# adelacvg/diff-vits

Measured on AMD Instinct MI355X. Metric: mel_frames_per_sec_50step_dpmsolver, higher is better.
Workload: dtype bf16x3 (bf16 MFMA operands split hi+lo, 3 products, fp32 accumulate / fp32 activations); 1 GPU; B=8/GPU, C=80, T=1024, L=256, 50-step DPM-Solver++(2M) multistep, UNet1DConditionModel (128, 256, 384, 512), seeded random-init weights; global_batch=8, concurrent_sub_batches_per_gpu=1, rccl_world_size=1, parallelism=dp1 (batch-sharded, RCCL broadcast of conditioning + all-gather of mels)

## Files before the change

diff-vits_amd/csrc/dv_common.h:

```cpp
#pragma once
#include <hip/hip_runtime.h>
#include <stdint.h>

typedef unsigned short bf16_t;

enum { DV_ZERO_PAGE_BYTES = 32768 };
enum { EPI_STORE = 0, EPI_RESIDUAL = 1, EPI_GEGLU = 2, EPI_STORE_NCT = 3 };
enum { UP_NONE = 0, UP_X2 = 1, UP_SIZE = 2 };

struct GemmSeg {
  const bf16_t* a0_hi; const bf16_t* a0_lo;
  const bf16_t* a1_hi; const bf16_t* a1_lo;
  int c0, c1;
  int taps;
  int pad;
  int nkt;
};

struct GnxParams {
  unsigned long long* xchg;
  unsigned* status;
  const float* gamma; const float* beta;
  const float* tscale; const float* tshift; int ld_t;
  int groups; float eps; int silu;
// ... 97 lines not shown
struct ChainFFParams {
  int M, C, T;
  int Tv;
  const bf16_t* a_hi; const bf16_t* a_lo;
  const float* rowstat; float ln_eps;
  const bf16_t* wg_hi; const bf16_t* wg_lo; const float* bg; const float* ug;
  const bf16_t* wm_hi; const bf16_t* wm_lo; const float* bm;
  const float* res;
  float* out; float* stats16;
  bf16_t* out_hi; bf16_t* out_lo;
  GnxParams gnx;
};
bool chain_ff_supported(const ChainFFParams& p, int precision);
int chain_ff_gnx_plan(const ChainFFParams& p, int n_cu);
hipError_t launch_chain_ff(const ChainFFParams& p, int precision, hipStream_t st);

struct FFSplitParams {
  int M, C, T;
  int rows;
  int Tv;
  int nspl;
  const bf16_t* a_hi; const bf16_t* a_lo;
  const float* rowstat; float ln_eps;
  const bf16_t* wg_hi; const bf16_t* wg_lo; const float* bg; const float* ug;
  const bf16_t* wm_hi; const bf16_t* wm_lo; const float* bm;
  const float* res;
  float* out; float* stats16;
  bf16_t* out_hi; bf16_t* out_lo;
  float* xbuf;
  unsigned long long* flags;
// ... 154 lines not shown
```

diff-vits_amd/csrc/engine.hip:

```cpp
#include "../../include/dvits_hip.h"
#include "dv_common.h"

#include <atomic>
#include <cmath>
#include <cstdarg>
#include <cstdio>
#include <cstdlib>
#include <cstring>
#include <functional>
#include <map>
#include <memory>
#include <string>
#include <type_traits>
#include <vector>

static thread_local char g_err[1024] = "";
int dv_fail(int code, const char* fmt, ...) {
  va_list ap;
  va_start(ap, fmt);
  vsnprintf(g_err, sizeof(g_err), fmt, ap);
  va_end(ap);
  return code;
}
extern "C" const char* dv_last_error(void) { return g_err; }
// ... 584 lines not shown
    Planes y, sy, sr;
    if (!gnx_offer(prod, nn, &y, &sy, &sr)) return;
    const bool cat = nn.skip.C > 0;
    out.n_hi = y.hi; out.n_lo = y.lo; out.n_pre = nn.pre;
    if (cat) { out.sn_hi = sy.hi; out.sn_lo = sy.lo; out.sr_hi = sr.hi; out.sr_lo = sr.lo; }
    const bool fp32_unread = cat && nn.raw && !u->keep_intermediates;
    if (nn.raw && !prod.out_hi) out_planes(prod, out);
    if (fp32_unread && cat_drop_fp32) prod.out = nullptr;
  }
  template <class P> void out_planes(P& prod, Act& out) {
    Planes pl = alloc_planes((size_t)prod.M * out.C);
    out.pl_hi = pl.hi; out.pl_lo = pl.lo; prod.out_hi = pl.hi; prod.out_lo = pl.lo;
  }
  bool ff_split_on = [] { const char* e = getenv("DVITS_FF_SPLIT"); return !(e && e[0] == '0'); }();
  bool chain_ff_on = [] { const char* e = getenv("DVITS_CHAIN_FF"); return !(e && e[0] == '0'); }();
  bool chain_split_on = [] { const char* e = getenv("DVITS_CHAIN_SPLIT"); return !(e && e[0] == '0'); }();
  bool chain_xsplit_on = [] { const char* e = getenv("DVITS_CHAIN_XSPLIT"); return !(e && e[0] == '0'); }();
  bool qkv_split_on = [] { const char* e = getenv("DVITS_QKV_SPLIT"); return !(e && e[0] == '0'); }();
  int qkv_split_min_wg = [] { const char* e = getenv("DVITS_QKV_SPLIT_MIN_WG"); return e ? atoi(e) : 96; }();
  int qkv_split_min_c = [] { const char* e = getenv("DVITS_QKV_SPLIT_MIN_C"); return e ? atoi(e) : 256; }();
  bool qkv_xa_on = [] { const char* e = getenv("DVITS_QKV_XA"); return !(e && e[0] == '0'); }();
  int qkv_xa_min_c = [] { const char* e = getenv("DVITS_QKV_XA_MIN_C"); return e ? atoi(e) : 256; }();
  int ff_split_min_wg = [] { const char* e = getenv("DVITS_FF_SPLIT_MIN_WG"); return e ? atoi(e) : 96; }();
  bool gnx_ff_on = [] { const char* e = getenv("DVITS_GNX_FF"); return !(e && e[0] == '0'); }();
  bool cat_drop_fp32 = [] { const char* e = getenv("DVITS_GNX_CONCAT_KEEP_FP32"); return !(e && e[0] == '1'); }();

  int conv3_min_tiles = [] { const char* e = getenv("DVITS_CONV3_MIN_TILES"); return e ? atoi(e) : 64; }();
  int conv3_route(const GemmParams& g) const {
    if (arena.exact || autotune_on() || prec != DV_PREC_BF16X3) return 0;
    GemmParams t = g;
// ... 338 lines not shown
    b.w_q2 = pack(tb + "q2", C, C, {{tb + "attn2.to_q.weight", 0, C, 1, C, 0, 0, tb + "norm2.weight", 0}},
                  {{"", "", tb + "attn2.to_q.weight", tb + "norm2.bias", C, C, 0, 0}});
    b.w_o2 = pack(tb + "out2", C, C, {{tb + "attn2.to_out.0.weight", 0, C, 1, C, 0, 0, "", 0}},
                  {{tb + "attn2.to_out.0.bias", "", "", "", C, 0, 0, 0}});
    b.w_gg = pack(tb + "geglu", 8 * C, C, {{tb + "ff.net.0.proj.weight", 0, C, 1, C, 0, 0, tb + "norm3.weight", 1}},
                  {{tb + "ff.net.0.proj.bias", "", tb + "ff.net.0.proj.weight", tb + "norm3.bias", 8 * C, C, 0, 1}});
    b.merged_ffproj = merge_ff && fuse_ln && !u->keep_intermediates;
    b.w_ff = b.merged_ffproj ? b.w_gg : pack(tb + "ffout", C, 4 * C, {{tb + "ff.net.2.weight", 0, 4 * C, 1, 4 * C, 0, 0, "", 0}},
                                             {{tb + "ff.net.2.bias", "", "", "", C, 0, 0, 0}});
    b.w_out = b.merged_ffproj ? b.w_gg : pack(p + "proj_out", C, C, {{p + "proj_out.weight", 1, C, 1, C, 0, 0, "", 0}},
                                              {{p + "proj_out.bias", "", "", "", C, 0, 0, 0}});
    if (!b.w_in || !b.w_qkv || !b.w_o1 || !b.w_q2 || !b.w_o2 || !b.w_gg || !b.w_ff || !b.w_out) return Act{};

    float* h3 = nullptr;
    LnIn l3;
    if (chain_ok(b.Tp, C) && x.stat16) {
      if (!(frag(b.w_in) && frag(b.w_qkv) && frag(b.w_o1) && frag(b.w_q2))) return Act{};
      float* h = nullptr;
      const Planes ao = xf_head(ops, b, h);
      if (!xf_tail(ops, b, h, ao, h3, l3)) return Act{};
    } else h3 = xf_attention_gemms(ops, b, l3);
    return xf_ff(ops, b, h3, l3, want_planes);
  }

  Planes xf_head(std::vector<OpFn>& ops, const Xf& b, float*& h) {
    const int C = b.C, Tn = b.Tn, Tp = b.Tp, M = b.M;
    h = alloc((size_t)M * C);
    const int dh = C / u->cfg.num_heads;
    const bool sa_frag = attn_frag_on && !arena.exact && C % u->cfg.num_heads == 0 && dh % 16 == 0 && dh <= 64;
    float* qkv = alloc((size_t)M * (sa_frag ? 1 : 3) * C);
    Planes kf, vf;
    if (sa_frag) { kf = alloc_planes((size_t)M * C); vf = alloc_planes((size_t)M * C); }
    ChainParams cp{};
    cp.M = M; cp.C = C; cp.T = Tp; cp.Tv = Tn; cp.amode = 1;
    cp.x = b.x.p; cp.stat16 = b.x.stat16; cp.gamma = W(b.p + "norm.weight"); cp.beta = W(b.p + "norm.bias"); cp.gn_eps = 1e-6f;
    cp.groups = u->cfg.norm_num_groups;
    cp.w1_hi = b.w_in->fhi; cp.w1_lo = b.w_in->flo; cp.Kp1 = b.w_in->Kp; cp.b1 = b.w_in->bias; cp.res = nullptr; cp.out1 = h;
// ... 14 lines not shown
    if (sa_frag) {
      AttnFragParams a{};
      a.q = qkv; a.ldq = C;
      a.kf_hi = kf.hi; a.kf_lo = kf.lo; a.vf_hi = vf.hi; a.vf_lo = vf.lo;
      const int nT = Tp / 32;
      a.k_b = nT * (C / 16); a.k_h = dh / 16; a.k_t = C / 16;
      a.v_b = nT * (C / 32) * 2; a.v_h = 0; a.v_t = (C / 32) * 2; a.v_kb = 1; a.v_nb = 2; a.self_layout = 1;
      a.bias = nullptr; a.bias_ld = 0;
      ao = attention_frag(ops, a, Tp, Tn, C);
      release(kf); release(vf);
    } else ao = attention(ops, qkv, 3 * C, qkv + C, qkv + 2 * C, 3 * C, nullptr, Tp, Tn, C, Tp);
    release(qkv);
    return ao;
  }

  bool xf_tail(std::vector<OpFn>& ops, const Xf& b, float* h, Planes ao, float*& h3, LnIn& l3) {
    const int C = b.C, M = b.M;
    if (xa_ok(b.Tp, C) && cross_frag.count(b.p)) {
      if (!frag(b.w_o2)) return false;
      float* h2 = alloc((size_t)M * C);
      h3 = alloc((size_t)M * C);
      l3 = ln_planes(M, C);
      xf_xattn_chain(ops, b, h, ao, h2, h3, l3);
      release(ao); release(h);
      probe(b.tb + "attn1", h2, b.Tn, C);
      release(h2);
      probe(b.tb + "attn2", h3, b.Tn, C);
      return true;
    }
    float* h2 = alloc((size_t)M * C);
    float* q2 = alloc((size_t)M * C);
    ChainParams cp = tail_chain(b, h, ao, h2);
    cp.out2 = q2;
    {
      const int rbs = M / 32, cus = n_cu > 0 ? n_cu : 256, nsg = C / 128;
      cp.nsplit = (chain_split_on && nsg >= 2 && rbs * nsg <= cus) ? nsg : 1;
    }
    const int n_qflags = qkv_split_flags(cp);
// ... 3 lines not shown
    if (!split) chain(ops, cp, "to_out+res+LN+to_q");
    release(ao); release(h);
    probe(b.tb + "attn1", h2, b.Tn, C);
    h3 = cross_attention_out(ops, b, q2, h2, l3);
    return true;
  }
  ChainParams tail_chain(const Xf& b, float* h, Planes ao, float* h2) {
    ChainParams cp{};
    cp.M = b.M; cp.C = b.C; cp.T = b.Tp; cp.Tv = b.Tn; cp.amode = 0;
    cp.a_hi = ao.hi; cp.a_lo = ao.lo;
    cp.w1_hi = b.w_o1->fhi; cp.w1_lo = b.w_o1->flo; cp.Kp1 = b.w_o1->Kp; cp.b1 = b.w_o1->bias; cp.res = h; cp.out1 = h2;
    cp.w2_hi = b.w_q2->fhi; cp.w2_lo = b.w_q2->flo; cp.Kp2 = b.w_q2->Kp; cp.b2 = b.w_q2->bias; cp.u2 = b.w_q2->u;
    cp.passes = 1; cp.out2 = nullptr; cp.ldo2 = b.C; cp.ln_eps = 1e-5f;
    return cp;
  }
  void xf_xattn_chain(std::vector<OpFn>& ops, const Xf& b, float* h, Planes ao, float* h2, float* h3, const LnIn& l3) {
    const int C = b.C, Tp = b.Tp, M = b.M;
    const XFrag& xf = cross_frag[b.p];
    ChainParams cp = tail_chain(b, h, ao, h2);
    cp.xa_kf_hi = xf.kf_hi; cp.xa_kf_lo = xf.kf_lo; cp.xa_vf_hi = xf.vf_hi; cp.xa_vf_lo = xf.vf_lo; cp.xa_bias = xbias;
    cp.xa_nT = (L + 31) / 32; cp.xa_d = C / u->cfg.num_heads;
    cp.xa_qscale = (1.0f / sqrtf((float)cp.xa_d)) * 1.44269504088896340736f;
    cp.w3_hi = b.w_o2->fhi; cp.w3_lo = b.w_o2->flo; cp.b3 = b.w_o2->bias;
    cp.out3 = h3; cp.out3_hi = l3.pl.hi; cp.out3_lo = l3.pl.lo; cp.rowstat3 = l3.stat;
    {
      const int rbs = M / 32, cus = n_cu > 0 ? n_cu : 256;
      if (chain_xsplit_on && C == 256 && rbs * 2 <= cus && rbs <= 4096 && (dry || u->sk_tickets)) {
        cp.nsplit = 2;
        cp.xs_buf = alloc((size_t)rbs * 2 * C * 32);
        cp.xs_ticket = dry ? reinterpret_cast<unsigned*>(0x1000) : u->sk_tickets;
      }
    }
    ChainParams cq = cp;
    cq.nsplit = 1; cq.xs_buf = nullptr; cq.xs_ticket = nullptr;
    const double xattn_flops = 4.0 * B * u->cfg.num_heads * (double)Tp * L * cp.xa_d + 2.0 * (double)M * C * C;
    const int n_wg = (M / 64) * (C / 64);
    bool split_xa = qkv_split_on && qkv_xa_on && C >= qkv_xa_min_c && handover_ok() && !autotune_on() &&
                    Tp % 64 == 0 && (M / 64) % 8 == 0 && n_wg <= n_cu && n_wg >= qkv_split_min_wg && u->cfg.num_heads == 8 &&
                    gnx_used + (size_t)2 * n_wg <= dv_unet::GNX_POOL;
    Planes oxa;
    if (split_xa) {
      oxa = alloc_planes((size_t)M * C);
      cq.qs_o_hi = oxa.hi; cq.qs_o_lo = oxa.lo;
      split_xa = qkv_split(ops, cq, strf("to_out+res+LN+to_q+xattn+to_out+res (%d wg / 64 rows) M=%d C=%d", C / 64, M, C), xattn_flops);
      if (!split_xa) release(oxa);
    }
    if (!split_xa)
      chain(ops, cp, cp.nsplit == 2 ? "to_out+res+LN+to_q+xattn(2 wg)+to_out+res" : "to_out+res+LN+to_q+xattn+to_out+res", xattn_flops);
    if (cp.xs_buf) release(cp.xs_buf);
    if (split_xa) release(oxa);
  }

  float* xf_attention_gemms(std::vector<OpFn>& ops, const Xf& b, LnIn& l3) {
    const int C = b.C, Tn = b.Tn, Tp = b.Tp, M = b.M;
    float* h = alloc((size_t)M * C);
    LnIn l1;
    {
      GemmParams g = gp_base(Tn, M, C);
      g.out = h; l1 = ln_produce(g, M, C);
      Planes gn;
      if (b.x.n_hi && b.x.n_pre == b.p + "norm") { gn.hi = b.x.n_hi; gn.lo = b.x.n_lo; }
// ... 36 lines not shown
    Planes ao;
    if (attn_frag_on && !arena.exact && cross_frag.count(b.p)) ao = cross_attention_frag(ops, b.p, q2, Tp, C);
    else ao = attention(ops, q2, C, kv, kv + C, 2 * C, mask_bias, Tp, L, C);
    release(q2);
    float* h3 = alloc((size_t)M * C);
    {
      GemmParams g = gp_base(b.Tn, M, C); g.seg[0] = seg(ao, C, Planes{}, 0, 1, 0);
      g.epi = EPI_RESIDUAL; g.res = h2; g.out = h3; l3 = ln_produce(g, M, C);
      gemm(ops, g, b.w_o2, C);
    }
    release(ao); release(h2);
    probe(b.tb + "attn2", h3, b.Tn, C);
    return h3;
  }

  Act xf_ff(std::vector<OpFn>& ops, const Xf& b, float* h3, LnIn& l3, bool want_planes) {
    const int C = b.C, Tp = b.Tp, M = b.M;
    const bool one_launch = b.merged_ffproj && chain_on && !arena.exact && l3.stat && b.x.stat16;
    ChainFFParams cf{};
    cf.M = M; cf.C = C; cf.T = Tp; cf.Tv = b.Tn;
    FFSplitParams fs{};
    fs.M = M; fs.C = C; fs.T = Tp; fs.Tv = b.Tn; fs.nspl = C == 256 ? 4 : 8;
    fs.rows = ff_split_rows(C, M, Tp, fs.nspl, n_cu);
    const int ff_wg = (M / fs.rows) * fs.nspl;
    const size_t n_flags = (size_t)ff_wg * 8;
    if (one_launch && chain_ff_on && chain_ff_supported(cf, prec)) return ff_launch(ops, b, cf, h3, l3, want_planes);
    else if (one_launch && ff_split_on && handover_ok() && !autotune_on() && (C == 256 || C == 384 || C == 512) &&
             ff_split_supported(fs, prec) && (ff_wg <= n_cu || gemm_handover_rounds()) && ff_wg >= ff_split_min_wg &&
             gnx_used + n_flags <= dv_unet::GNX_POOL)
      return ff_launch(ops, b, fs, h3, l3, want_planes);
    else return xf_ff_gemms(ops, b, h3, l3, want_planes);
  }
  const PackedW* ffproj_weight(const Xf& b) {
    const int C = b.C;
    const std::string &p = b.p, &tb = b.tb;
    const std::string mw = tb + "__ffproj.weight", mb = tb + "__ffproj.bias";
    if (!dry && !u->packed.count(p + "ffproj")) {
      const float* Wo = W(p + "proj_out.weight"); const float* W2 = W(tb + "ff.net.2.weight");
      const float* bo = W(p + "proj_out.bias"); const float* b2 = W(tb + "ff.net.2.bias");
      float* dw = derived(mw, {C, 4 * C});
      float* db = derived(mb, {C});
      if (!Wo || !W2 || !bo || !b2 || !dw || !db) return nullptr;
      (void)launch_matmul_f32(Wo, W2, dw, C, C, 4 * C, pack_stream);
      (void)launch_fold_bias(Wo, bo, b2, db, C, C, 0, 0, pack_stream);
    }
    return pack(p + "ffproj", C, 5 * C, {{p + "proj_out.weight", 1, C, 1, C, 0, 0, "", 0}, {mw, 0, 4 * C, 1, 4 * C, C, 0, "", 0}},
                {{mb, "", "", "", C, 0, 0, 0}});
  }
  template <class FF> Act ff_launch(std::vector<OpFn>& ops, const Xf& b, FF fp, float* h3, LnIn& l3, bool want_planes) {
    constexpr bool split = std::is_same<FF, FFSplitParams>::value;
    const int C = b.C, M = b.M;
    const PackedW* w_m = ffproj_weight(b);
    if (!w_m || !frag(b.w_gg) || !frag(w_m)) return Act{};
    Act out{};
    out.p = alloc((size_t)M * C); out.C = C; out.T = b.Tn; out.Tp = b.Tp; alloc_stat(out, true);
    fp.a_hi = l3.pl.hi; fp.a_lo = l3.pl.lo; fp.rowstat = l3.stat; fp.ln_eps = 1e-5f;
    fp.wg_hi = b.w_gg->fhi; fp.wg_lo = b.w_gg->flo; fp.bg = b.w_gg->bias; fp.ug = b.w_gg->u;
    fp.wm_hi = w_m->fhi; fp.wm_lo = w_m->flo; fp.bm = w_m->bias;
    fp.res = b.x.p; fp.out = out.p; fp.stats16 = out.stat16;
    if constexpr (split) {
      const Handover ho = handover((size_t)(M / fp.rows) * fp.nspl * 8);
      fp.flags = ho.flags; fp.status = ho.status; fp.spin_max = gnx_spin;
      fp.xbuf = alloc(ff_split_xbuf_floats(M, C, fp.nspl, fp.rows));
    }
    if (want_planes) out_planes(fp, out);
    offer_next(fp, out);
    const double flops = 2.0 * (double)M * C * (8.0 * C + 5.0 * C);
    const char* gnx = fp.gnx.xchg ? "+gnx" : "";
    const int pr = prec;
    if constexpr (split) {
      emit_launch(ops, "chain", flops, strf("LN+GEGLU+ffproj+res%s (%d wg / %d rows) M=%d C=%d", gnx, fp.nspl, fp.rows, M, C),
                  [fp, pr](hipStream_t st) { return launch_ff_split(fp, pr, st); });
      release(fp.xbuf);
    } else {
      emit_launch(ops, "chain", flops, strf("LN+GEGLU+ffproj+res%s M=%d C=%d", gnx, M, C),
                  [fp, pr](hipStream_t st) { return launch_chain_ff(fp, pr, st); });
    }
    ln_release(l3);
    release(h3);
    probe(b.p.substr(0, b.p.size() - 1), out.p, b.Tn, C);
    return out;
  }
  Act xf_ff_gemms(std::vector<OpFn>& ops, const Xf& b, float* h3, LnIn& l3, bool want_planes) {
    const int C = b.C, Tn = b.Tn, Tp = b.Tp, M = b.M;
    Planes gg = alloc_planes((size_t)M * 4 * C);
    {
      GemmParams g = gp_base(Tn, M, 8 * C);
      g.epi = EPI_GEGLU; g.out_hi = gg.hi; g.out_lo = gg.lo; g.ldo = 4 * C; ln_consume(ops, g, l3, h3, b.w_gg, M, C); gemm(ops, g, b.w_gg, C);
    }
    if (b.merged_ffproj) {
      const PackedW* w_m = ffproj_weight(b);
      if (!w_m) return Act{};
      Act out{};
      out.p = alloc((size_t)M * C); out.C = C; out.T = Tn; out.Tp = Tp; alloc_stat(out);
// ... 1196 lines not shown
```

diff-vits_amd/csrc/kernels_chain.hip:

```cpp
#include "dv_common.h"
#include "dv_device.h"
#include "gnx_device.h"

#include <cstdlib>
#include <type_traits>

typedef __attribute__((ext_vector_type(8))) __bf16 bf16x8;
typedef __attribute__((ext_vector_type(16))) float f32x16;

#ifdef DV_GEMM_TRACE
__device__ unsigned long long g_chain_trace[8192 * 16];
__device__ int g_chain_sel[3] = {0, -1, -1};
#define DV_CTRACE(i) do { if (threadIdx.x == 0 && blockIdx.x < 8192 && (g_chain_sel[0] == 0 || g_chain_sel[0] == p.C) && \
    (g_chain_sel[1] < 0 || g_chain_sel[1] == p.amode) && (g_chain_sel[2] < 0 || g_chain_sel[2] == (p.xa_kf_hi != nullptr))) \
    g_chain_trace[blockIdx.x * 16 + (i)] = __builtin_amdgcn_s_memtime(); } while (0)
extern "C" int dv_debug_chain_trace_select(int C, int amode, int xa) {
  const int h[3] = {C, amode, xa};
  hipError_t e = hipMemcpyToSymbol(HIP_SYMBOL(g_chain_sel), h, sizeof(h));
  void* d = nullptr;
  if (e == hipSuccess) e = hipGetSymbolAddress(&d, HIP_SYMBOL(g_chain_trace));
  return (int)(e != hipSuccess ? e : hipMemset(d, 0, sizeof(g_chain_trace)));
}
extern "C" int dv_debug_chain_trace(unsigned long long* host, int n_wg) {
  return (int)hipMemcpyFromSymbol(host, HIP_SYMBOL(g_chain_trace), (size_t)n_wg * 16 * sizeof(unsigned long long));
// ... 13 lines not shown
constexpr int DEPTH_FF = DV_DEPTH_FF;

__device__ __forceinline__ int swz(int row) { return (row >> 1) & 7; }
__device__ __forceinline__ unsigned pk(float lo, float hi) { return dv_cvt_pk_bf16(lo, hi); }

#ifndef DV_CHAIN_PFMODE
#define DV_CHAIN_PFMODE 2
#endif
template <int NS, int AMODE, bool XA, bool SA, bool CS>
constexpr bool chain_pf_wave() {
  if (XA) return false;
  if (DV_CHAIN_PFMODE == 0) return !(SA && NS >= 3);
  return NS == 1 || (NS == 2 && AMODE == 0);
}

template <int NS, int AMODE, bool XA = false, bool SA = false, bool CS = false>
__global__ __launch_bounds__((chain_pf_wave<NS, AMODE, XA, SA, CS>() ? NT_LAUNCH : NT)) void k_chain2(const ChainParams p) {
  extern __shared__ __attribute__((aligned(1024))) char smem[];
  constexpr int CH = 2 * NS;
  constexpr int A_PL = CH * CHUNK_PL;
  constexpr int C = 128 * NS;
  constexpr bool PFW = chain_pf_wave<NS, AMODE, XA, SA, CS>();
  char* const a_reg = smem;
  char* const red_reg = smem + 2 * A_PL;
  __shared__ float2 s_rowp[BM][16];
  __shared__ __attribute__((aligned(16))) float2 s_ln[BM];
  __shared__ __attribute__((aligned(16))) float s_gscale[AMODE ? C : 4], s_gshift[AMODE ? C : 4];
  __shared__ __attribute__((aligned(256))) unsigned s_pf[64];

  asm volatile("" ::"s"(p.M), "s"(p.gamma), "s"(p.w1_lo), "s"(p.out1), "s"(p.u2), "s"(p.xa_kf_hi), "s"(p.xa_bias), "s"(p.w3_lo),
               "s"(p.out3_lo), "s"(p.sa_vf_lo), "s"(p.nsplit));
  const int tid = threadIdx.x, lane = tid & 63, wave = __builtin_amdgcn_readfirstlane(tid >> 6);
  auto l2_prefetch = [&](int w, int nw) __attribute__((always_inline)) {
// ... 574 lines not shown
      }
    }
    if (kg == 0) {
      const int m = m0 + l31;
#pragma unroll
      for (int ns = 0; ns < NS; ++ns) {
        const int nf = ns * 128 + wn * 32 + 4 * lh;
        float vv[16];
#pragma unroll
        for (int g = 0; g < 4; ++g) {
          const float4 bv = *reinterpret_cast<const float4*>(p.b3 + nf + 8 * g);
          const float4 rr = *reinterpret_cast<const float4*>(p.out1 + (size_t)m * C + nf + 8 * g);
          vv[4 * g] = acc[ns][4 * g] + bv.x + rr.x; vv[4 * g + 1] = acc[ns][4 * g + 1] + bv.y + rr.y;
          vv[4 * g + 2] = acc[ns][4 * g + 2] + bv.z + rr.z; vv[4 * g + 3] = acc[ns][4 * g + 3] + bv.w + rr.w;
        }
#pragma unroll
        for (int g = 0; g < 4; ++g)
          dv_st16(p.out3 + (size_t)m * C + nf + 8 * g, make_float4(vv[4 * g], vv[4 * g + 1], vv[4 * g + 2], vv[4 * g + 3]));
        store_planes16(p.out3_hi, p.out3_lo, (size_t)m * C + nf - 4 * lh, lh, vv);
        float a = 0.f, q = 0.f;
#pragma unroll
        for (int r = 0; r < 16; ++r) a += vv[r];
        a = pair_sum32(a);
        const float mb = a * (1.0f / 32.0f);
#pragma unroll
        for (int r = 0; r < 16; ++r) q += (vv[r] - mb) * (vv[r] - mb);
        q = pair_sum32(q);
        if (lh == 0) reinterpret_cast<float2*>(p.rowstat3)[(size_t)m * (C / 32) + ns * 4 + wn] = make_float2(a, q);
      }
    }
  }
  DV_CTRACE(9);
}

__global__ __launch_bounds__(NT_LAUNCH) void k_chain_ff(const ChainFFParams p) {
  extern __shared__ __attribute__((aligned(1024))) char smem[];
  constexpr int C = 128, A_CH = 2, G_CH = 8;
  constexpr int A_PL = A_CH * CHUNK_PL, G_PL = G_CH * CHUNK_PL;
  char* const a_reg = smem;
  char* const g_reg = smem + 2 * A_PL;
  char* const red_reg = g_reg + 2 * G_PL;
  __shared__ __attribute__((aligned(16))) float2 s_ln[BM];
  asm volatile("" ::"s"(p.M), "s"(p.rowstat), "s"(p.wg_lo), "s"(p.wm_hi), "s"(p.res), "s"(p.out_lo));
  const int tid = threadIdx.x, lane = tid & 63, wave = __builtin_amdgcn_readfirstlane(tid >> 6);
  if (wave == NWV) {
    __shared__ __attribute__((aligned(256))) unsigned s_pf[64];
    const int xw = blockIdx.x >> 3, nxw = (gridDim.x + 7) >> 3;
    const int lg = 8 * C * C / 64, lm = 5 * C * C / 64;
    const int total = 2 * (lg + lm), per = (total + nxw - 1) / nxw, end = min(total, (xw + 1) * per);
    for (int ln = xw * per + lane; ln < end; ln += 64) {
      const char* src;
      if (ln < lg) src = reinterpret_cast<const char*>(p.wg_hi) + (size_t)ln * 128;
      else if (ln < 2 * lg) src = reinterpret_cast<const char*>(p.wg_lo) + (size_t)(ln - lg) * 128;
      else if (ln < 2 * lg + lm) src = reinterpret_cast<const char*>(p.wm_hi) + (size_t)(ln - 2 * lg) * 128;
      else src = reinterpret_cast<const char*>(p.wm_lo) + (size_t)(ln - 2 * lg - lm) * 128;
      glds4(src, (unsigned)(size_t)s_pf);
    }
    const char* r0 = reinterpret_cast<const char*>(p.res + (size_t)blockIdx.x * BM * C);
    for (int ln = lane; ln < BM * C / 32; ln += 64) glds4(r0 + (size_t)ln * 128, (unsigned)(size_t)s_pf);
    for (int ln = lane; ln < 8 * C / 32; ln += 64) {
      glds4(reinterpret_cast<const char*>(p.bg) + (size_t)ln * 128, (unsigned)(size_t)s_pf);
      glds4(reinterpret_cast<const char*>(p.ug) + (size_t)ln * 128, (unsigned)(size_t)s_pf);
    }
    return;
  }
  const int l31 = lane & 31, lh = lane >> 5;
  const int m0 = blockIdx.x * BM;
  const unsigned a_base = (unsigned)(size_t)a_reg;
  const int d_row = lane >> 3, d_slot = lane & 7;
  struct BFrag { bf16x8 h, l; };

  for (int idx = wave; idx < A_CH * 4; idx += NWV) {
    const int c = idx >> 2, r8 = idx & 3, row = r8 * 8 + d_row;
    const size_t e = (size_t)(m0 + row) * C + c * 64 + ((d_slot ^ swz(row)) << 3);
    const unsigned dst = a_base + (unsigned)(c * CHUNK_PL + r8 * 1024);
    glds16(p.a_hi + e, dst);
    glds16(p.a_lo + e, dst + A_PL);
  }
  constexpr int UA = 32;
  auto load_a_unit = [&](int U) __attribute__((always_inline)) {
    const int nf = 2 * ((U >> 4) * 8 + wave) + (U & 1), ks = (U & 15) >> 1;
    const size_t e = ((size_t)(nf * 8 + ks) * 64 + lane) * 8;
    BFrag f;
    f.h = *reinterpret_cast<const bf16x8*>(p.wg_hi + e);
    f.l = *reinterpret_cast<const bf16x8*>(p.wg_lo + e);
    return f;
  };
  BFrag bq[DEPTH_FF];
#pragma unroll
  for (int j = 0; j < DEPTH_FF; ++j) bq[j] = load_a_unit(j);
  __builtin_amdgcn_sched_barrier(0);
  if (tid < BM) {
    const float2* src = reinterpret_cast<const float2*>(p.rowstat) + (size_t)(m0 + tid) * (C / 32);
    float2 v[C / 32];
#pragma unroll
    for (int k = 0; k < C / 32; ++k) v[k] = src[k];
    float s1 = 0.f;
#pragma unroll
    for (int k = 0; k < C / 32; ++k) s1 += v[k].x;
    const float inv_c = 1.0f / (float)C, mean = s1 * inv_c;
    float m2 = 0.f;
#pragma unroll
    for (int k = 0; k < C / 32; ++k) { const float dm = v[k].x * (1.0f / 32.0f) - mean; m2 += v[k].y + 32.0f * dm * dm; }
    s_ln[tid] = make_float2(mean, 1.0f / sqrtf(m2 * inv_c + p.ln_eps));
  }
  wait_vmcnt<0>();
  __syncthreads();

  {
    auto read_a = [&](int ks, bf16x8& h, bf16x8& l) __attribute__((always_inline)) {
      const int c16 = ks * 2 + lh;
      const int off = (c16 >> 3) * CHUNK_PL + l31 * 128 + (((c16 & 7) ^ swz(l31)) << 4);
      h = *reinterpret_cast<const bf16x8*>(a_reg + off);
      l = *reinterpret_cast<const bf16x8*>(a_reg + A_PL + off);
    };
    const float2 st = s_ln[l31];
#pragma unroll
    for (int ps = 0; ps < 2; ++ps) {
      f32x16 acc[2];
#pragma unroll
      for (int f = 0; f < 2; ++f)
#pragma unroll
        for (int r = 0; r < 16; ++r) acc[f][r] = 0.f;
      bf16x8 ah, al;
#pragma unroll
      for (int uu = 0; uu < 16; ++uu) {
        const int U = ps * 16 + uu;
        if ((uu & 1) == 0) read_a(uu >> 1, ah, al);
        const BFrag f = bq[U % DEPTH_FF];
        acc[uu & 1] = __builtin_amdgcn_mfma_f32_32x32x16_bf16(f.h, al, acc[uu & 1], 0, 0, 0);
        acc[uu & 1] = __builtin_amdgcn_mfma_f32_32x32x16_bf16(f.l, ah, acc[uu & 1], 0, 0, 0);
// ... 137 lines not shown
      for (int g = 0; g < 4; ++g) {
        const float4 sa = *reinterpret_cast<const float4*>(s_gnx.gA + nf + 8 * g);
        const float4 sb = *reinterpret_cast<const float4*>(s_gnx.gB + nf + 8 * g);
        y[4 * g] = fmaf(vv[4 * g], sa.x, sb.x); y[4 * g + 1] = fmaf(vv[4 * g + 1], sa.y, sb.y);
        y[4 * g + 2] = fmaf(vv[4 * g + 2], sa.z, sb.z); y[4 * g + 3] = fmaf(vv[4 * g + 3], sa.w, sb.w);
      }
      if (p.gnx.silu) {
#pragma unroll
        for (int r = 0; r < 16; ++r) y[r] = y[r] * __builtin_amdgcn_rcpf(1.0f + __expf(-y[r]));
      }
      store_planes16(p.gnx.y_hi, p.gnx.y_lo, (size_t)m * C + nf - 4 * lh, lh, y);
    }
  }
}

__global__ __launch_bounds__(64) void k_kv_frag(const float* __restrict__ kv, bf16_t* __restrict__ kf_hi, bf16_t* __restrict__ kf_lo,
                                                bf16_t* __restrict__ vf_hi, bf16_t* __restrict__ vf_lo, int L, int C, int H, int nT) {
  const int t = blockIdx.x, h = blockIdx.y, b = blockIdx.z, lane = threadIdx.x, l31 = lane & 31, lh = lane >> 5;
  const int d = C / H, KSq = d >> 4, NBv = (d + 31) >> 5;
  const size_t bh = (size_t)b * H + h;
  auto split8 = [&](const float (&v)[8], bf16_t* hi, bf16_t* lo) {
    uint4 hw, lw;
    unsigned* hp = &hw.x; unsigned* lp = &lw.x;
#pragma unroll
    for (int e = 0; e < 4; ++e) {
      const unsigned h2 = pk(v[2 * e], v[2 * e + 1]);
      hp[e] = h2;
      lp[e] = pk(v[2 * e] - __uint_as_float(h2 << 16), v[2 * e + 1] - __uint_as_float(h2 & 0xffff0000u));
    }
    *reinterpret_cast<uint4*>(hi) = hw;
// ... 69 lines not shown
}
hipError_t launch_chain_ff(const ChainFFParams& p, int precision, hipStream_t st) {
  if (!chain_ff_supported(p, precision)) return hipErrorInvalidValue;
  if (!p.a_hi || !p.a_lo || !p.rowstat || !p.wg_hi || !p.wg_lo || !p.bg || !p.ug || !p.wm_hi || !p.wm_lo || !p.bm || !p.res ||
      (p.out_hi && !p.out_lo))
    return hipErrorInvalidValue;
  if (p.gnx.xchg) {
    static const int n_cu = [] { int d = 0, n = 0; (void)hipGetDevice(&d); (void)hipDeviceGetAttribute(&n, hipDeviceAttributeMultiprocessorCount, d); return n; }();
    if (!p.gnx.status || !p.gnx.y_hi || !p.gnx.y_lo || !p.gnx.gamma || !p.gnx.beta || chain_ff_gnx_plan(p, n_cu) <= 0) return hipErrorInvalidValue;
    if (p.gnx.sk_c > 0 && (!p.gnx.sk_x || !p.gnx.sk_stat16 || !p.gnx.sk_y_hi || !p.gnx.sk_y_lo)) return hipErrorInvalidValue;
  } else if (!p.out) return hipErrorInvalidValue;
  hipLaunchKernelGGL(k_chain_ff, dim3(p.M / BM), dim3(NT_LAUNCH), FF_SMEM, st, p);
  return hipGetLastError();
}

hipError_t chain_init() {
  hipError_t e;
  if ((e = hipFuncSetAttribute(reinterpret_cast<const void*>(k_chain_ff), hipFuncAttributeMaxDynamicSharedMemorySize, FF_SMEM)) != hipSuccess) return e;
  if ((e = init_one<1, 0>()) != hipSuccess) return e;
  if ((e = init_one<2, 0>()) != hipSuccess) return e;
  if ((e = init_one<3, 0>()) != hipSuccess) return e;
  if ((e = init_one<1, 1>()) != hipSuccess) return e;
  if ((e = init_one<2, 1>()) != hipSuccess) return e;
  if ((e = init_one<3, 1>()) != hipSuccess) return e;
  if ((e = init_one<1, 1, false, true>()) != hipSuccess) return e;
  if ((e = init_one<2, 1, false, true>()) != hipSuccess) return e;
  if ((e = init_one<3, 1, false, true>()) != hipSuccess) return e;
  if ((e = init_one<2, 0, false, false, true>()) != hipSuccess) return e;
  if ((e = init_one<3, 0, false, false, true>()) != hipSuccess) return e;
  if ((e = init_one<1, 0, true>()) != hipSuccess) return e;
  if ((e = init_one<2, 0, true, false, true>()) != hipSuccess) return e;
  return init_one<2, 0, true>();
// ... 66 lines not shown
```

Baseline: 68210 mel-frames/s.

## Fuse C=128 cross-attention chain with feed-forward chain into one kernel

Adds k_chain_xff, which runs the to_out+res+LN+to_q+xattn+to_out+res chain and then the LN+GEGLU+ffproj+res chain in the same workgroup. The intermediate residual is handed to the FF stage as bf16 hi/lo planes in LDS, and the LN row partials go through shared memory, so the fp32 h3 write, its planes and the rowstat round trip through global memory disappear, along with one launch per transformer block at C=128. In exchange the fused kernel loses the dedicated prefetch wave and the FF launch's wider block, and it stacks both stages' LDS and register pressure in a single kernel.

```diff
diff --git a/diff-vits_amd/csrc/dv_common.h b/diff-vits_amd/csrc/dv_common.h
--- a/diff-vits_amd/csrc/dv_common.h
+++ b/diff-vits_amd/csrc/dv_common.h
@@ -135,6 +135,9 @@
 bool chain_ff_supported(const ChainFFParams& p, int precision);
 int chain_ff_gnx_plan(const ChainFFParams& p, int n_cu);
 hipError_t launch_chain_ff(const ChainFFParams& p, int precision, hipStream_t st);
+struct ChainXffParams { ChainParams c; ChainFFParams f; };
+bool chain_xff_supported(const ChainXffParams& p, int precision);
+hipError_t launch_chain_xff(const ChainXffParams& p, int precision, hipStream_t st);
 
 struct FFSplitParams {
   int M, C, T;
diff --git a/diff-vits_amd/csrc/engine.hip b/diff-vits_amd/csrc/engine.hip
--- a/diff-vits_amd/csrc/engine.hip
+++ b/diff-vits_amd/csrc/engine.hip
@@ -622,6 +622,14 @@
   }
   bool ff_split_on = [] { const char* e = getenv("DVITS_FF_SPLIT"); return !(e && e[0] == '0'); }();
   bool chain_ff_on = [] { const char* e = getenv("DVITS_CHAIN_FF"); return !(e && e[0] == '0'); }();
+  bool chain_xff_on = [] { const char* e = getenv("DVITS_CHAIN_XFF"); return !(e && e[0] == '0'); }();
+  struct XffPark {
+    bool armed = false;
+    ChainParams cp{};
+    double flops = 0;
+    Planes ao;
+    float *h = nullptr, *h2 = nullptr;
+  };
   bool chain_split_on = [] { const char* e = getenv("DVITS_CHAIN_SPLIT"); return !(e && e[0] == '0'); }();
   bool chain_xsplit_on = [] { const char* e = getenv("DVITS_CHAIN_XSPLIT"); return !(e && e[0] == '0'); }();
   bool qkv_split_on = [] { const char* e = getenv("DVITS_QKV_SPLIT"); return !(e && e[0] == '0'); }();
@@ -990,13 +998,14 @@
 
     float* h3 = nullptr;
     LnIn l3;
+    XffPark park;
     if (chain_ok(b.Tp, C) && x.stat16) {
       if (!(frag(b.w_in) && frag(b.w_qkv) && frag(b.w_o1) && frag(b.w_q2))) return Act{};
       float* h = nullptr;
       const Planes ao = xf_head(ops, b, h);
-      if (!xf_tail(ops, b, h, ao, h3, l3)) return Act{};
+      if (!xf_tail(ops, b, h, ao, h3, l3, park)) return Act{};
     } else h3 = xf_attention_gemms(ops, b, l3);
-    return xf_ff(ops, b, h3, l3, want_planes);
+    return xf_ff(ops, b, h3, l3, want_planes, park);
   }
 
   Planes xf_head(std::vector<OpFn>& ops, const Xf& b, float*& h) {
@@ -1041,14 +1050,20 @@
     return ao;
   }
 
-  bool xf_tail(std::vector<OpFn>& ops, const Xf& b, float* h, Planes ao, float*& h3, LnIn& l3) {
+  bool xf_tail(std::vector<OpFn>& ops, const Xf& b, float* h, Planes ao, float*& h3, LnIn& l3, XffPark& park) {
     const int C = b.C, M = b.M;
     if (xa_ok(b.Tp, C) && cross_frag.count(b.p)) {
       if (!frag(b.w_o2)) return false;
       float* h2 = alloc((size_t)M * C);
+      park.armed = chain_xff_on && C == 128 && qkv_xa_min_c > C && C / u->cfg.num_heads == 16 && ff_is_chain(b, true);
+      if (park.armed) {
+        xf_xattn_chain(ops, b, h, ao, h2, nullptr, LnIn{}, &park);
+        park.ao = ao; park.h = h; park.h2 = h2;
+        return true;
+      }
       h3 = alloc((size_t)M * C);
       l3 = ln_planes(M, C);
-      xf_xattn_chain(ops, b, h, ao, h2, h3, l3);
+      xf_xattn_chain(ops, b, h, ao, h2, h3, l3, nullptr);
       release(ao); release(h);
       probe(b.tb + "attn1", h2, b.Tn, C);
       release(h2);
@@ -1082,7 +1097,7 @@
     cp.passes = 1; cp.out2 = nullptr; cp.ldo2 = b.C; cp.ln_eps = 1e-5f;
     return cp;
   }
-  void xf_xattn_chain(std::vector<OpFn>& ops, const Xf& b, float* h, Planes ao, float* h2, float* h3, const LnIn& l3) {
+  void xf_xattn_chain(std::vector<OpFn>& ops, const Xf& b, float* h, Planes ao, float* h2, float* h3, const LnIn& l3, XffPark* park) {
     const int C = b.C, Tp = b.Tp, M = b.M;
     const XFrag& xf = cross_frag[b.p];
     ChainParams cp = tail_chain(b, h, ao, h2);
@@ -1113,6 +1128,7 @@
       split_xa = qkv_split(ops, cq, strf("to_out+res+LN+to_q+xattn+to_out+res (%d wg / 64 rows) M=%d C=%d", C / 64, M, C), xattn_flops);
       if (!split_xa) release(oxa);
     }
+    if (park) { park->cp = cp; park->flops = chain_flops(cp) + xattn_flops; return; }
     if (!split_xa)
       chain(ops, cp, cp.nsplit == 2 ? "to_out+res+LN+to_q+xattn(2 wg)+to_out+res" : "to_out+res+LN+to_q+xattn+to_out+res", xattn_flops);
     if (cp.xs_buf) release(cp.xs_buf);
@@ -1179,9 +1195,15 @@
     return h3;
   }
 
-  Act xf_ff(std::vector<OpFn>& ops, const Xf& b, float* h3, LnIn& l3, bool want_planes) {
+  bool ff_one_launch(const Xf& b, bool ln_partials) const { return b.merged_ffproj && chain_on && !arena.exact && ln_partials && b.x.stat16; }
+  bool ff_is_chain(const Xf& b, bool ln_partials) const {
+    ChainFFParams cf{};
+    cf.M = b.M; cf.C = b.C; cf.T = b.Tp; cf.Tv = b.Tn;
+    return ff_one_launch(b, ln_partials) && chain_ff_on && chain_ff_supported(cf, prec);
+  }
+  Act xf_ff(std::vector<OpFn>& ops, const Xf& b, float* h3, LnIn& l3, bool want_planes, const XffPark& park) {
     const int C = b.C, Tp = b.Tp, M = b.M;
-    const bool one_launch = b.merged_ffproj && chain_on && !arena.exact && l3.stat && b.x.stat16;
+    const bool one_launch = ff_one_launch(b, l3.stat || park.armed);
     ChainFFParams cf{};
     cf.M = M; cf.C = C; cf.T = Tp; cf.Tv = b.Tn;
     FFSplitParams fs{};
@@ -1189,11 +1211,12 @@
     fs.rows = ff_split_rows(C, M, Tp, fs.nspl, n_cu);
     const int ff_wg = (M / fs.rows) * fs.nspl;
     const size_t n_flags = (size_t)ff_wg * 8;
-    if (one_launch && chain_ff_on && chain_ff_supported(cf, prec)) return ff_launch(ops, b, cf, h3, l3, want_planes);
-    else if (one_launch && ff_split_on && handover_ok() && !autotune_on() && (C == 256 || C == 384 || C == 512) &&
+    if (ff_is_chain(b, l3.stat || park.armed)) return ff_launch(ops, b, cf, h3, l3, want_planes, &park);
+    if (park.armed) { err = "k_chain_xff: the feed-forward did not take the parked chain"; return Act{}; }
+    if (one_launch && ff_split_on && handover_ok() && !autotune_on() && (C == 256 || C == 384 || C == 512) &&
              ff_split_supported(fs, prec) && (ff_wg <= n_cu || gemm_handover_rounds()) && ff_wg >= ff_split_min_wg &&
              gnx_used + n_flags <= dv_unet::GNX_POOL)
-      return ff_launch(ops, b, fs, h3, l3, want_planes);
+      return ff_launch(ops, b, fs, h3, l3, want_planes, nullptr);
     else return xf_ff_gemms(ops, b, h3, l3, want_planes);
   }
   const PackedW* ffproj_weight(const Xf& b) {
@@ -1212,7 +1235,7 @@
     return pack(p + "ffproj", C, 5 * C, {{p + "proj_out.weight", 1, C, 1, C, 0, 0, "", 0}, {mw, 0, 4 * C, 1, 4 * C, C, 0, "", 0}},
                 {{mb, "", "", "", C, 0, 0, 0}});
   }
-  template <class FF> Act ff_launch(std::vector<OpFn>& ops, const Xf& b, FF fp, float* h3, LnIn& l3, bool want_planes) {
+  template <class FF> Act ff_launch(std::vector<OpFn>& ops, const Xf& b, FF fp, float* h3, LnIn& l3, bool want_planes, const XffPark* park) {
     constexpr bool split = std::is_same<FF, FFSplitParams>::value;
     const int C = b.C, M = b.M;
     const PackedW* w_m = ffproj_weight(b);
@@ -1238,11 +1261,19 @@
                   [fp, pr](hipStream_t st) { return launch_ff_split(fp, pr, st); });
       release(fp.xbuf);
     } else {
-      emit_launch(ops, "chain", flops, strf("LN+GEGLU+ffproj+res%s M=%d C=%d", gnx, M, C),
-                  [fp, pr](hipStream_t st) { return launch_chain_ff(fp, pr, st); });
+      if (park && park->armed) {
+        const ChainXffParams xp{park->cp, fp};
+        if (!dry && !chain_xff_supported(xp, pr)) {
+          err = "k_chain_xff does not take the planned launch"; return Act{}; }
+        emit_launch(ops, "chain", park->flops + flops, strf("LN+GEGLU+ffproj+res%s behind to_out+res+LN+to_q+xattn+to_out+res M=%d C=%d", gnx, M, C),
+                    [xp, pr](hipStream_t st) { return launch_chain_xff(xp, pr, st); });
+        release(park->ao); release(park->h); release(park->h2);
+      } else
+        emit_launch(ops, "chain", flops, strf("LN+GEGLU+ffproj+res%s M=%d C=%d", gnx, M, C),
+                    [fp, pr](hipStream_t st) { return launch_chain_ff(fp, pr, st); });
     }
     ln_release(l3);
-    release(h3);
+    if (h3) release(h3);
     probe(b.p.substr(0, b.p.size() - 1), out.p, b.Tn, C);
     return out;
   }
diff --git a/diff-vits_amd/csrc/kernels_chain.hip b/diff-vits_amd/csrc/kernels_chain.hip
--- a/diff-vits_amd/csrc/kernels_chain.hip
+++ b/diff-vits_amd/csrc/kernels_chain.hip
@@ -51,9 +51,36 @@
   return NS == 1 || (NS == 2 && AMODE == 0);
 }
 
-template <int NS, int AMODE, bool XA = false, bool SA = false, bool CS = false>
-__global__ __launch_bounds__((chain_pf_wave<NS, AMODE, XA, SA, CS>() ? NT_LAUNCH : NT)) void k_chain2(const ChainParams p) {
-  extern __shared__ __attribute__((aligned(1024))) char smem[];
+__device__ __forceinline__ void ff_l2_prefetch(const ChainFFParams& p, unsigned* s_pf, int lane, int w, int nw) {
+  constexpr int C = 128;
+  const int xw = blockIdx.x >> 3, nxw = (gridDim.x + 7) >> 3;
+  const int lg = 8 * C * C / 64, lm = 5 * C * C / 64;
+  const int total = 2 * (lg + lm), per = (total + nxw - 1) / nxw, end = min(total, (xw + 1) * per);
+  for (int ln = xw * per + w * 64 + lane; ln < end; ln += 64 * nw) {
+    const char* src;
+    if (ln < lg) src = reinterpret_cast<const char*>(p.wg_hi) + (size_t)ln * 128;
+    else if (ln < 2 * lg) src = reinterpret_cast<const char*>(p.wg_lo) + (size_t)(ln - lg) * 128;
+    else if (ln < 2 * lg + lm) src = reinterpret_cast<const char*>(p.wm_hi) + (size_t)(ln - 2 * lg) * 128;
+    else src = reinterpret_cast<const char*>(p.wm_lo) + (size_t)(ln - 2 * lg - lm) * 128;
+    glds4(src, (unsigned)(size_t)s_pf);
+  }
+  const char* r0 = reinterpret_cast<const char*>(p.res + (size_t)blockIdx.x * BM * C);
+  for (int ln = w * 64 + lane; ln < BM * C / 32; ln += 64 * nw) glds4(r0 + (size_t)ln * 128, (unsigned)(size_t)s_pf);
+  if (w == 0)
+    for (int ln = lane; ln < 8 * C / 32; ln += 64) {
+      glds4(reinterpret_cast<const char*>(p.bg) + (size_t)ln * 128, (unsigned)(size_t)s_pf);
+      glds4(reinterpret_cast<const char*>(p.ug) + (size_t)ln * 128, (unsigned)(size_t)s_pf);
+    }
+}
+
+struct XffSeam {
+  char* a_img;
+  float2 (*rowp)[4];
+};
+
+template <int NS, int AMODE, bool XA, bool SA, bool CS, bool XFF>
+__device__ __forceinline__ void chain2_body(const ChainParams& p, char* const smem, const XffSeam seam) {
+  static_assert(!XFF || (XA && NS == 1 && !CS && !SA && AMODE == 0), "the fused form exists for the C = 128 cross-attention chain");
   constexpr int CH = 2 * NS;
   constexpr int A_PL = CH * CHUNK_PL;
   constexpr int C = 128 * NS;
@@ -658,10 +685,25 @@
           vv[4 * g] = acc[ns][4 * g] + bv.x + rr.x; vv[4 * g + 1] = acc[ns][4 * g + 1] + bv.y + rr.y;
           vv[4 * g + 2] = acc[ns][4 * g + 2] + bv.z + rr.z; vv[4 * g + 3] = acc[ns][4 * g + 3] + bv.w + rr.w;
         }
-#pragma unroll
-        for (int g = 0; g < 4; ++g)
-          dv_st16(p.out3 + (size_t)m * C + nf + 8 * g, make_float4(vv[4 * g], vv[4 * g + 1], vv[4 * g + 2], vv[4 * g + 3]));
-        store_planes16(p.out3_hi, p.out3_lo, (size_t)m * C + nf - 4 * lh, lh, vv);
+        if constexpr (XFF) {
+#pragma unroll
+          for (int g = 0; g < 4; ++g) {
+            const int n = nf + 8 * g;
+            uint2 hw, lw;
+            hw.x = pk(vv[4 * g], vv[4 * g + 1]); hw.y = pk(vv[4 * g + 2], vv[4 * g + 3]);
+            lw.x = pk(vv[4 * g] - __uint_as_float(hw.x << 16), vv[4 * g + 1] - __uint_as_float(hw.x & 0xffff0000u));
+            lw.y = pk(vv[4 * g + 2] - __uint_as_float(hw.y << 16), vv[4 * g + 3] - __uint_as_float(hw.y & 0xffff0000u));
+            const int c = n >> 6, s16 = (n & 63) >> 3;
+            const int off = c * CHUNK_PL + l31 * 128 + ((s16 ^ swz(l31)) << 4) + ((n & 7) >> 2) * 8;
+            *reinterpret_cast<uint2*>(seam.a_img + off) = hw;
+            *reinterpret_cast<uint2*>(seam.a_img + A_PL + off) = lw;
+          }
+        } else {
+#pragma unroll
+          for (int g = 0; g < 4; ++g)
+            dv_st16(p.out3 + (size_t)m * C + nf + 8 * g, make_float4(vv[4 * g], vv[4 * g + 1], vv[4 * g + 2], vv[4 * g + 3]));
+          store_planes16(p.out3_hi, p.out3_lo, (size_t)m * C + nf - 4 * lh, lh, vv);
+        }
         float a = 0.f, q = 0.f;
 #pragma unroll
         for (int r = 0; r < 16; ++r) a += vv[r];
@@ -670,15 +712,34 @@
 #pragma unroll
         for (int r = 0; r < 16; ++r) q += (vv[r] - mb) * (vv[r] - mb);
         q = pair_sum32(q);
-        if (lh == 0) reinterpret_cast<float2*>(p.rowstat3)[(size_t)m * (C / 32) + ns * 4 + wn] = make_float2(a, q);
+        if constexpr (XFF) { if (lh == 0) seam.rowp[l31][ns * 4 + wn] = make_float2(a, q); }
+        else if (lh == 0) reinterpret_cast<float2*>(p.rowstat3)[(size_t)m * (C / 32) + ns * 4 + wn] = make_float2(a, q);
       }
     }
   }
   DV_CTRACE(9);
 }
 
-__global__ __launch_bounds__(NT_LAUNCH) void k_chain_ff(const ChainFFParams p) {
+template <int NS, int AMODE, bool XA = false, bool SA = false, bool CS = false>
+__global__ __launch_bounds__((chain_pf_wave<NS, AMODE, XA, SA, CS>() ? NT_LAUNCH : NT)) void k_chain2(const ChainParams p) {
   extern __shared__ __attribute__((aligned(1024))) char smem[];
+  chain2_body<NS, AMODE, XA, SA, CS, false>(p, smem, XffSeam{nullptr, nullptr});
+}
+
+__device__ __forceinline__ float2 ln_finish128(const float2 (&v)[4], float eps) {
+  constexpr int C = 128;
+  float s1 = 0.f;
+#pragma unroll
+  for (int k = 0; k < C / 32; ++k) s1 += v[k].x;
+  const float inv_c = 1.0f / (float)C, mean = s1 * inv_c;
+  float m2 = 0.f;
+#pragma unroll
+  for (int k = 0; k < C / 32; ++k) { const float dm = v[k].x * (1.0f / 32.0f) - mean; m2 += v[k].y + 32.0f * dm * dm; }
+  return make_float2(mean, 1.0f / sqrtf(m2 * inv_c + eps));
+}
+
+template <bool FUSED>
+__device__ __forceinline__ void chain_ff_body(const ChainFFParams& p, char* const smem, const float2 (*rowp)[4]) {
   constexpr int C = 128, A_CH = 2, G_CH = 8;
   constexpr int A_PL = A_CH * CHUNK_PL, G_PL = G_CH * CHUNK_PL;
   char* const a_reg = smem;
@@ -687,25 +748,9 @@
   __shared__ __attribute__((aligned(16))) float2 s_ln[BM];
   asm volatile("" ::"s"(p.M), "s"(p.rowstat), "s"(p.wg_lo), "s"(p.wm_hi), "s"(p.res), "s"(p.out_lo));
   const int tid = threadIdx.x, lane = tid & 63, wave = __builtin_amdgcn_readfirstlane(tid >> 6);
-  if (wave == NWV) {
+  if (!FUSED && wave == NWV) {
     __shared__ __attribute__((aligned(256))) unsigned s_pf[64];
-    const int xw = blockIdx.x >> 3, nxw = (gridDim.x + 7) >> 3;
-    const int lg = 8 * C * C / 64, lm = 5 * C * C / 64;
-    const int total = 2 * (lg + lm), per = (total + nxw - 1) / nxw, end = min(total, (xw + 1) * per);
-    for (int ln = xw * per + lane; ln < end; ln += 64) {
-      const char* src;
-      if (ln < lg) src = reinterpret_cast<const char*>(p.wg_hi) + (size_t)ln * 128;
-      else if (ln < 2 * lg) src = reinterpret_cast<const char*>(p.wg_lo) + (size_t)(ln - lg) * 128;
-      else if (ln < 2 * lg + lm) src = reinterpret_cast<const char*>(p.wm_hi) + (size_t)(ln - 2 * lg) * 128;
-      else src = reinterpret_cast<const char*>(p.wm_lo) + (size_t)(ln - 2 * lg - lm) * 128;
-      glds4(src, (unsigned)(size_t)s_pf);
-    }
-    const char* r0 = reinterpret_cast<const char*>(p.res + (size_t)blockIdx.x * BM * C);
-    for (int ln = lane; ln < BM * C / 32; ln += 64) glds4(r0 + (size_t)ln * 128, (unsigned)(size_t)s_pf);
-    for (int ln = lane; ln < 8 * C / 32; ln += 64) {
-      glds4(reinterpret_cast<const char*>(p.bg) + (size_t)ln * 128, (unsigned)(size_t)s_pf);
-      glds4(reinterpret_cast<const char*>(p.ug) + (size_t)ln * 128, (unsigned)(size_t)s_pf);
-    }
+    ff_l2_prefetch(p, s_pf, lane, 0, 1);
     return;
   }
   const int l31 = lane & 31, lh = lane >> 5;
@@ -714,13 +759,14 @@
   const int d_row = lane >> 3, d_slot = lane & 7;
   struct BFrag { bf16x8 h, l; };
 
-  for (int idx = wave; idx < A_CH * 4; idx += NWV) {
-    const int c = idx >> 2, r8 = idx & 3, row = r8 * 8 + d_row;
-    const size_t e = (size_t)(m0 + row) * C + c * 64 + ((d_slot ^ swz(row)) << 3);
-    const unsigned dst = a_base + (unsigned)(c * CHUNK_PL + r8 * 1024);
-    glds16(p.a_hi + e, dst);
-    glds16(p.a_lo + e, dst + A_PL);
-  }
+  if (!FUSED)
+    for (int idx = wave; idx < A_CH * 4; idx += NWV) {
+      const int c = idx >> 2, r8 = idx & 3, row = r8 * 8 + d_row;
+      const size_t e = (size_t)(m0 + row) * C + c * 64 + ((d_slot ^ swz(row)) << 3);
+      const unsigned dst = a_base + (unsigned)(c * CHUNK_PL + r8 * 1024);
+      glds16(p.a_hi + e, dst);
+      glds16(p.a_lo + e, dst + A_PL);
+    }
   constexpr int UA = 32;
   auto load_a_unit = [&](int U) __attribute__((always_inline)) {
     const int nf = 2 * ((U >> 4) * 8 + wave) + (U & 1), ks = (U & 15) >> 1;
@@ -734,21 +780,16 @@
 #pragma unroll
   for (int j = 0; j < DEPTH_FF; ++j) bq[j] = load_a_unit(j);
   __builtin_amdgcn_sched_barrier(0);
-  if (tid < BM) {
-    const float2* src = reinterpret_cast<const float2*>(p.rowstat) + (size_t)(m0 + tid) * (C / 32);
-    float2 v[C / 32];
-#pragma unroll
-    for (int k = 0; k < C / 32; ++k) v[k] = src[k];
-    float s1 = 0.f;
-#pragma unroll
-    for (int k = 0; k < C / 32; ++k) s1 += v[k].x;
-    const float inv_c = 1.0f / (float)C, mean = s1 * inv_c;
-    float m2 = 0.f;
-#pragma unroll
-    for (int k = 0; k < C / 32; ++k) { const float dm = v[k].x * (1.0f / 32.0f) - mean; m2 += v[k].y + 32.0f * dm * dm; }
-    s_ln[tid] = make_float2(mean, 1.0f / sqrtf(m2 * inv_c + p.ln_eps));
-  }
-  wait_vmcnt<0>();
+  if (!FUSED) {
+    if (tid < BM) {
+      const float2* src = reinterpret_cast<const float2*>(p.rowstat) + (size_t)(m0 + tid) * (C / 32);
+      float2 v[C / 32];
+#pragma unroll
+      for (int k = 0; k < C / 32; ++k) v[k] = src[k];
+      s_ln[tid] = ln_finish128(v, p.ln_eps);
+    }
+    wait_vmcnt<0>();
+  }
   __syncthreads();
 
   {
@@ -758,7 +799,13 @@
       h = *reinterpret_cast<const bf16x8*>(a_reg + off);
       l = *reinterpret_cast<const bf16x8*>(a_reg + A_PL + off);
     };
-    const float2 st = s_ln[l31];
+    float2 st;
+    if (FUSED) {
+      float2 v[C / 32];
+#pragma unroll
+      for (int k = 0; k < C / 32; ++k) v[k] = rowp[l31][k];
+      st = ln_finish128(v, p.ln_eps);
+    } else st = s_ln[l31];
 #pragma unroll
     for (int ps = 0; ps < 2; ++ps) {
       f32x16 acc[2];
@@ -926,6 +973,19 @@
   }
 }
 
+__global__ __launch_bounds__(NT_LAUNCH) void k_chain_ff(const ChainFFParams p) {
+  extern __shared__ __attribute__((aligned(1024))) char smem[];
+  chain_ff_body<false>(p, smem, nullptr);
+}
+
+constexpr int XFF_CHAIN_OFF = 2 * 2 * CHUNK_PL;
+__global__ __launch_bounds__(NT) void k_chain_xff(const ChainXffParams p) {
+  extern __shared__ __attribute__((aligned(1024))) char smem[];
+  __shared__ __attribute__((aligned(16))) float2 s_rowp3[BM][4];
+  chain2_body<1, 0, true, false, false, true>(p.c, smem + XFF_CHAIN_OFF, XffSeam{smem, s_rowp3});
+  chain_ff_body<true>(p.f, smem, s_rowp3);
+}
+
 __global__ __launch_bounds__(64) void k_kv_frag(const float* __restrict__ kv, bf16_t* __restrict__ kf_hi, bf16_t* __restrict__ kf_lo,
                                                 bf16_t* __restrict__ vf_hi, bf16_t* __restrict__ vf_lo, int L, int C, int H, int nT) {
   const int t = blockIdx.x, h = blockIdx.y, b = blockIdx.z, lane = threadIdx.x, l31 = lane & 31, lh = lane >> 5;
@@ -1025,8 +1085,32 @@
   return hipGetLastError();
 }
 
+bool chain_xff_supported(const ChainXffParams& p, int precision) {
+  const ChainParams& c = p.c;
+  ChainParams t = c;
+  t.out3 = t.out1; t.rowstat3 = t.out1; t.out3_hi = t.out3_lo = reinterpret_cast<bf16_t*>(t.out1);
+  if (!chain2_supported(t, precision) || !chain_ff_supported(p.f, precision)) return false;
+  if (c.C != 128 || !c.xa_kf_hi || c.xa_d != 16 || c.amode != 0 || c.nsplit > 1) return false;
+  return c.M == p.f.M && c.T == p.f.T && c.Tv == p.f.Tv;
+}
+hipError_t launch_chain_xff(const ChainXffParams& p, int precision, hipStream_t st) {
+  if (!chain_xff_supported(p, precision)) return hipErrorInvalidValue;
+  const ChainParams& c = p.c;
+  const ChainFFParams& f = p.f;
+  if (!c.a_hi || !c.a_lo || !c.w1_hi || !c.w1_lo || !c.w2_hi || !c.w2_lo || !c.b1 || !c.b2 || !c.u2 || !c.out1) return hipErrorInvalidValue;
+  if (!f.wg_hi || !f.wg_lo || !f.bg || !f.ug || !f.wm_hi || !f.wm_lo || !f.bm || !f.res || (f.out_hi && !f.out_lo)) return hipErrorInvalidValue;
+  if (f.gnx.xchg) {
+    static const int n_cu = [] { int d = 0, n = 0; (void)hipGetDevice(&d); (void)hipDeviceGetAttribute(&n, hipDeviceAttributeMultiprocessorCount, d); return n; }();
+    if (!f.gnx.status || !f.gnx.y_hi || !f.gnx.y_lo || !f.gnx.gamma || !f.gnx.beta || chain_ff_gnx_plan(f, n_cu) <= 0) return hipErrorInvalidValue;
+    if (f.gnx.sk_c > 0 && (!f.gnx.sk_x || !f.gnx.sk_stat16 || !f.gnx.sk_y_hi || !f.gnx.sk_y_lo)) return hipErrorInvalidValue;
+  } else if (!f.out) return hipErrorInvalidValue;
+  hipLaunchKernelGGL(k_chain_xff, dim3(f.M / BM), dim3(NT), FF_SMEM, st, p);
+  return hipGetLastError();
+}
+
 hipError_t chain_init() {
   hipError_t e;
+  if ((e = hipFuncSetAttribute(reinterpret_cast<const void*>(k_chain_xff), hipFuncAttributeMaxDynamicSharedMemorySize, FF_SMEM)) != hipSuccess) return e;
   if ((e = hipFuncSetAttribute(reinterpret_cast<const void*>(k_chain_ff), hipFuncAttributeMaxDynamicSharedMemorySize, FF_SMEM)) != hipSuccess) return e;
   if ((e = init_one<1, 0>()) != hipSuccess) return e;
   if ((e = init_one<2, 0>()) != hipSuccess) return e;
```

Result: no change. 68890 mel-frames/s (median of 6 runs) (+1.0%).
